# ApproximateCaesar/AlphaQuoridorGNN

Hardware: AMD Instinct MI355X
Metric: self-play games/sec, 9x9 Quoridor (PV-MCTS, GNN evaluator), whole job (higher is better)
Workload: dtype f32 (f16x3-split MFMA products, f32 accumulate); 1 GPU; BASELINE configs[2]/[3]: one self-play generation per step (lock-step PV-MCTS, random-weight GNN) + all-gather of (s,pi,z); games_per_gpu=2048, game_sets_per_gpu=4, sims_per_move=200, board=9x9, walls=10, plies_for_draw=116, parallelism=games sharded over 1 rank(s), 1 all-gather per generation

## Files before the change

### alphaquoridorgnn_amd/csrc/gcn_heads_split.hpp

```cpp
#pragma once
#include "gcn_packed.hpp"
#include <cmath>

namespace aqg {

__device__ __forceinline__ float row16_sum(float x) {
    x += __builtin_bit_cast(float, __builtin_amdgcn_update_dpp(0, __builtin_bit_cast(int, x), 0x128, 0xf, 0xf, false));
    x += __builtin_bit_cast(float, __builtin_amdgcn_update_dpp(0, __builtin_bit_cast(int, x), 0x124, 0xf, 0xf, false));
    x += __builtin_bit_cast(float, __builtin_amdgcn_update_dpp(0, __builtin_bit_cast(int, x), 0x122, 0xf, 0xf, false));
    x += __builtin_bit_cast(float, __builtin_amdgcn_update_dpp(0, __builtin_bit_cast(int, x), 0x121, 0xf, 0xf, false));
    return x;
}

__device__ __forceinline__ __amdgpu_buffer_rsrc_t packed_rsrc(const float* pk) {
    return __builtin_amdgcn_make_buffer_rsrc(const_cast<float*>(pk), 0, (int)(PackedLayout::TOTAL * sizeof(float)), 0x00020000);
}
__device__ __forceinline__ u32x4 load_frag16(__amdgpu_buffer_rsrc_t rs, int lane16, int byte_off) {
    return __builtin_amdgcn_raw_buffer_load_b128(rs, lane16, byte_off, 0);
}

__device__ __forceinline__ void report_saturation(bool lane_saw_it, int32_t* __restrict__ saturated) {
    if (saturated && __builtin_amdgcn_ballot_w64(lane_saw_it) != 0) {
        int l;
        asm volatile("v_mbcnt_lo_u32_b32 %0, -1, 0\n\tv_mbcnt_hi_u32_b32 %0, -1, %0" : "=v"(l));
        if (l == 0) atomicOr(saturated, 1);
    }
}

__device__ __forceinline__ void split8(const f32x4 x0, const f32x4 x1, u32x4& hi, u32x4& lo) {
    hi = (u32x4){cvt_pk_f16(x0[0], x0[1]), cvt_pk_f16(x0[2], x0[3]), cvt_pk_f16(x1[0], x1[1]), cvt_pk_f16(x1[2], x1[3])};
    const f32x4 r0 = x0 - f16_pairs_to_f32(hi[0], hi[1]), r1 = x1 - f16_pairs_to_f32(hi[2], hi[3]);
    lo = (u32x4){cvt_pk_f16(r0[0], r0[1]), cvt_pk_f16(r0[2], r0[3]), cvt_pk_f16(r1[0], r1[1]), cvt_pk_f16(r1[2], r1[3])};
}
__device__ __forceinline__ float row16_max(float x) {
    x = fmaxf(x, __builtin_bit_cast(float, __builtin_amdgcn_update_dpp(0, __builtin_bit_cast(int, x), 0x128, 0xf, 0xf, false)));
    x = fmaxf(x, __builtin_bit_cast(float, __builtin_amdgcn_update_dpp(0, __builtin_bit_cast(int, x), 0x124, 0xf, 0xf, false)));
    x = fmaxf(x, __builtin_bit_cast(float, __builtin_amdgcn_update_dpp(0, __builtin_bit_cast(int, x), 0x122, 0xf, 0xf, false)));
    x = fmaxf(x, __builtin_bit_cast(float, __builtin_amdgcn_update_dpp(0, __builtin_bit_cast(int, x), 0x121, 0xf, 0xf, false)));
    return x;
}

constexpr int HEADS_WAVES = 8;
struct alignas(16) HeadsSmem {
    unsigned int hfrag[2][2][64][4];
    float vlane[4][64];
    float wmax[HEADS_WAVES][16], wsum[HEADS_WAVES][16];
};

struct HeadsNoMid { __device__ __forceinline__ void operator()() const {} };
template <bool STEP = false, class Mid = HeadsNoMid>
__device__ __forceinline__ void heads_body(HeadsSmem& sm, __amdgpu_buffer_rsrc_t prs, int b0, int B, int A, __amdgpu_buffer_rsrc_t rs,
                                           const float* __restrict__ pk, float* __restrict__ logits, float* __restrict__ policy,
                                           float* __restrict__ value_pre, float* __restrict__ value, const uint8_t* __restrict__ active,
                                           int32_t* __restrict__ saturated, int wave, int lane, float (*lds_policy)[256] = nullptr,
                                           float* lds_value = nullptr, Mid mid = Mid()) {
    const int c = lane & 15, q = lane >> 4;
    constexpr int H1 = (int)(PackedLayout::WHH1 * sizeof(float)), P2 = (int)(PackedLayout::WHP2 * sizeof(float));
    const int ntiles = (A + 15) >> 4;
    const bool want_policy = STEP || logits || policy;
    u32x4 af[2][4];
#pragma unroll
    for (int pl = 0; pl < 2; ++pl)
#pragma unroll
        for (int kb = 0; kb < 4; ++kb) af[pl][kb] = load_frag16(rs, lane * 16, H1 + ((pl * 8 + wave) * 4 + kb) * (64 * 16));
    const bool okc = b0 + c < B;
    f32x4 x0[4], x1[4];
    {
        const int row = (okc ? b0 + c : B - 1) * (HID * 4);
#pragma unroll
        for (int kb = 0; kb < 4; ++kb) {
            x0[kb] = __builtin_bit_cast(f32x4, __builtin_amdgcn_raw_buffer_load_b128(prs, row + (32 * kb + 8 * q) * 4, 0, 0));
            x1[kb] = __builtin_bit_cast(f32x4, __builtin_amdgcn_raw_buffer_load_b128(prs, row + (32 * kb + 8 * q + 4) * 4, 0, 0));
        }
    }
    const f32x4 bias = *reinterpret_cast<const f32x4*>(pk + PackedLayout::HB1 + 16 * wave + 4 * q);
    const f32x4 vw = *reinterpret_cast<const f32x4*>(pk + PackedLayout::VW2 + 16 * (wave & 3) + 4 * q);
    float pb[2];
#pragma unroll
    for (int j = 0; j < 2; ++j) { const int a = 16 * (wave + 8 * j) + c; pb[j] = pk[PackedLayout::PB2 + (a < A ? a : 0)]; }
    const float vb2 = pk[PackedLayout::VB2];
    const uint8_t* __restrict__ ap = active ? active : reinterpret_cast<const uint8_t*>(pk);
    unsigned int af4[4];
#pragma unroll
    for (int i = 0; i < 4; ++i) af4[i] = ap[active ? min(b0 + 4 * q + i, B - 1) : 0];
    const unsigned int afc = ap[active ? min(b0 + c, B - 1) : 0];
    u32x4 ph[4], pl_[4];
    bool counted;
    {
        float xmax = 0.f;
#pragma unroll
        for (int kb = 0; kb < 4; ++kb) {
            if (!okc) { x0[kb] = (f32x4){0.f, 0.f, 0.f, 0.f}; x1[kb] = x0[kb]; }
#pragma unroll
            for (int e = 0; e < 4; ++e) xmax = fmaxf(fmaxf(fabsf(x0[kb][e]), fabsf(x1[kb][e])), xmax);
            split8(x0[kb], x1[kb], ph[kb], pl_[kb]);
        }
        counted = okc && (!active || (STEP ? afc == 1 : afc != 0));
        if (wave == 0) report_saturation(counted && !(xmax <= 65504.0f), saturated);
    }
    int live4 = 0;
#pragma unroll
    for (int i = 0; i < 4; ++i) live4 |= (b0 + 4 * q + i < B && (!active || (STEP ? af4[i] == 1 : af4[i] != 0))) ? (1 << i) : 0;
    u32x4 bq[2][2][2];
    auto request_bq = [&](int j, int kb) {
        const int at = wave + 8 * j;
#pragma unroll
        for (int pl = 0; pl < 2; ++pl)
            bq[j][pl][kb] = (want_policy && at < ntiles) ? load_frag16(rs, lane * 16, P2 + ((pl * 14 + at) * 2 + kb) * (64 * 16)) : (u32x4){0u, 0u, 0u, 0u};
    };
    if (!STEP) {
#pragma unroll
        for (int j = 0; j < 2; ++j)
#pragma unroll
            for (int kb = 0; kb < 2; ++kb) request_bq(j, kb);
    }
    {
        f32x4 acc = (f32x4){0.f, 0.f, 0.f, 0.f};
#pragma unroll
        for (int kb = 0; kb < 4; ++kb) {
            acc = mfma_f16(af[1][kb], ph[kb], acc);
            acc = mfma_f16(af[0][kb], pl_[kb], acc);
            acc = mfma_f16(af[0][kb], ph[kb], acc);
            if (STEP) {
                __builtin_amdgcn_sched_barrier(0);
                request_bq(kb >> 1, kb & 1);
                __builtin_amdgcn_sched_barrier(0);
            }
        }
        if (STEP) {
            __builtin_amdgcn_sched_barrier(0);
            mid();
            __builtin_amdgcn_sched_barrier(0);
        }
        f32x4 h = acc + bias;
#pragma unroll
        for (int e = 0; e < 4; ++e) h[e] = fmaxf(h[e], 0.f);
        if (wave < 4) {
            report_saturation(counted && !(fmaxf(fmaxf(h[0], h[1]), fmaxf(h[2], h[3])) <= 65504.0f), saturated);
            const unsigned int h01 = cvt_pk_f16(h[0], h[1]), h23 = cvt_pk_f16(h[2], h[3]);
            const f32x4 r = h - f16_pairs_to_f32(h01, h23);
            const int kb2 = wave >> 1, t = wave & 1;
            *reinterpret_cast<u32x2*>(&sm.hfrag[kb2][0][lane][2 * t]) = (u32x2){h01, h23};
            *reinterpret_cast<u32x2*>(&sm.hfrag[kb2][1][lane][2 * t]) = (u32x2){cvt_pk_f16(r[0], r[1]), cvt_pk_f16(r[2], r[3])};
        } else {
            sm.vlane[wave - 4][lane] = h[0] * vw[0] + h[1] * vw[1] + h[2] * vw[2] + h[3] * vw[3];
        }
    }
    __syncthreads();
    if (wave == 4) {
        float v = (sm.vlane[0][lane] + sm.vlane[1][lane]) + (sm.vlane[2][lane] + sm.vlane[3][lane]);
        v += __shfl_xor(v, 16);
        v += __shfl_xor(v, 32);
        if (counted && lane < 16) {
            v += vb2;
            if (STEP) lds_value[lane] = tanhf(v);
            else {
                if (value_pre) value_pre[b0 + lane] = v;
                if (value) value[b0 + lane] = tanhf(v);
            }
        }
    }
    if (!want_policy) return;
    u32x4 hh[2], hl[2];
#pragma unroll
    for (int kb = 0; kb < 2; ++kb) {
        hh[kb] = *reinterpret_cast<const u32x4*>(&sm.hfrag[kb][0][lane][0]);
        hl[kb] = *reinterpret_cast<const u32x4*>(&sm.hfrag[kb][1][lane][0]);
    }
    f32x4 lg[2];
    f32x4 m = (f32x4){-INFINITY, -INFINITY, -INFINITY, -INFINITY};
#pragma unroll
    for (int j = 0; j < 2; ++j) {
        const int at = wave + 8 * j, a = 16 * at + c;
        f32x4 acc = (f32x4){0.f, 0.f, 0.f, 0.f};
#pragma unroll
        for (int kb = 0; kb < 2; ++kb) {
            acc = mfma_f16(hl[kb], bq[j][0][kb], acc);
            acc = mfma_f16(hh[kb], bq[j][1][kb], acc);
            acc = mfma_f16(hh[kb], bq[j][0][kb], acc);
        }
        const bool ok = a < A;
#pragma unroll
        for (int i = 0; i < 4; ++i) {
            lg[j][i] = ok ? acc[i] + pb[j] : -INFINITY;
            m[i] = fmaxf(m[i], lg[j][i]);
        }
    }
    f32x4 ssum = (f32x4){0.f, 0.f, 0.f, 0.f};
    f32x4 ex[2];
#pragma unroll
    for (int i = 0; i < 4; ++i) m[i] = row16_max(m[i]);
#pragma unroll
    for (int j = 0; j < 2; ++j)
#pragma unroll
        for (int i = 0; i < 4; ++i) {
            ex[j][i] = __expf(lg[j][i] - m[i]);
            ssum[i] += ex[j][i];
        }
#pragma unroll
    for (int i = 0; i < 4; ++i) ssum[i] = row16_sum(ssum[i]);
    if (c == 0) {
        *reinterpret_cast<f32x4*>(&sm.wmax[wave][4 * q]) = m;
        *reinterpret_cast<f32x4*>(&sm.wsum[wave][4 * q]) = ssum;
    }
    __syncthreads();
    f32x4 scale;
    {
        int qo = 4 * q;
        f32x4 M = (f32x4){-INFINITY, -INFINITY, -INFINITY, -INFINITY};
#pragma unroll
        for (int w = 0; w < HEADS_WAVES; ++w) {
            const f32x4 mw = *reinterpret_cast<const f32x4*>(&sm.wmax[w][qo]);
#pragma unroll
            for (int i = 0; i < 4; ++i) M[i] = fmaxf(M[i], mw[i]);
        }
        f32x4 S = (f32x4){0.f, 0.f, 0.f, 0.f};
#pragma unroll
        for (int w = 0; w < HEADS_WAVES; ++w) {
            if (STEP && (w & 3) == 0) {
                const float d0 = w ? S[0] : M[0], d1 = w ? S[1] : M[1], d2 = w ? S[2] : M[2], d3 = w ? S[3] : M[3];
                asm volatile("" : "+v"(qo) : "v"(d0), "v"(d1), "v"(d2), "v"(d3));
            }
            const f32x4 mw = *reinterpret_cast<const f32x4*>(&sm.wmax[w][qo]);
            const f32x4 sw = *reinterpret_cast<const f32x4*>(&sm.wsum[w][qo]);
#pragma unroll
            for (int i = 0; i < 4; ++i) S[i] += sw[i] * __expf(mw[i] - M[i]);
        }
#pragma unroll
        for (int i = 0; i < 4; ++i) scale[i] = __expf(m[i] - M[i]) / S[i];
    }
#pragma unroll
    for (int i = 0; i < 4; ++i) {
        const int brd = b0 + 4 * q + i;
        if (!((live4 >> i) & 1)) continue;
        if (STEP) {
            float* p = &lds_policy[4 * q + i][16 * wave + c];
#pragma unroll
            for (int j = 0; j < 2; ++j) if (16 * (wave + 8 * j) + c < A) p[128 * j] = ex[j][i] * scale[i];
            continue;
        }
        const size_t row = (size_t)brd * A + 16 * wave + c;
        if (policy) {
            float* __restrict__ p = policy + row;
#pragma unroll
            for (int j = 0; j < 2; ++j) if (16 * (wave + 8 * j) + c < A) p[128 * j] = ex[j][i] * scale[i];
        }
        if (logits) {
            float* __restrict__ l = logits + row;
#pragma unroll
            for (int j = 0; j < 2; ++j) if (16 * (wave + 8 * j) + c < A) l[128 * j] = lg[j][i];
        }
    }
}

}
```

### alphaquoridorgnn_amd/csrc/mcts.hip

```cpp
#define AQG_TRACE_TU mcts
#include "aqg_common.hpp"
#include <vector>
#include <cstring>
#include "legal_wave.hpp"
#include "../../include/aqgnn.h"
#include "launchers.hpp"
#include "counter_rng.hpp"
#include "gcn_heads_split.hpp"
#include <cfloat>

#pragma clang fp contract(off)

namespace aqg {

int g_use_graph = 1;

__device__ __forceinline__ int wave_sum_i(int v) {
#pragma unroll
    for (int off = 32; off > 0; off >>= 1) v += __shfl_xor(v, off);
    return v;
}
__device__ __forceinline__ float wave_sum_f(float v) {
#pragma unroll
    for (int off = 32; off > 0; off >>= 1) v += __shfl_xor(v, off);
// ... 158 lines not shown
    const uint8_t* ord = e.legal_order + (size_t)g * MAX_LEGAL;
    const int prow = s.ppos / N;
    int rl[3]; int tot = 0;
#pragma unroll
    for (int r = 0; r < 3; ++r) {
        const int i = lane + 64 * r;
        rl[r] = 0;
        if (i < cnt) {
            const int a = ord[i];
            uint32_t x = ((h ^ ((uint32_t)(a + 1) * 0x9E3779B1u)) * 0x85EBCA6Bu) >> 22;
            int rr = (int)x + 1;
            if (a < V && (a / N) < prow) rr *= 1 + e.fake_bias;
            rl[r] = rr; tot += rr;
        }
    }
    tot = wave_sum_i(tot);
    float* pol = e.policy + (size_t)g * A;
#pragma unroll
    for (int r = 0; r < 3; ++r) {
        const int i = lane + 64 * r;
        if (i < cnt) pol[i] = (float)rl[r] / (float)tot;
    }
    if (lane == 0) e.value[g] = (float)((int)((h * 0xC2B2AE35u) >> 16) - 32768) / 32768.0f;
}

#ifdef AQG_STAMP
#define STEP_STAMP_DECL unsigned long long sp_prev = __builtin_readcyclecounter(), sp_loc[5] = {0, 0, 0, 0, 0};
#define STEP_STAMP(i) { const unsigned long long sp_now = __builtin_readcyclecounter(); if (lane == 0) reinterpret_cast<unsigned long long*>(e.pooled + (size_t)g * 128)[i] += sp_now - sp_prev; sp_loc[i] = sp_now - sp_prev; sp_prev = sp_now; }
#define LEVEL_STAMP(i) { const unsigned long long lv_now = __builtin_readcyclecounter(); if (lane == 0) reinterpret_cast<unsigned long long*>(e.pooled + (size_t)g * 128)[i] += lv_now - lv_prev; lv_prev = lv_now; }
#else
#define STEP_STAMP_DECL
#define STEP_STAMP(i)
#endif
constexpr int EVAL_CACHE_ROW = 704;
static_assert(MAX_LEGAL * 5 <= EVAL_CACHE_ROW && MAX_LEGAL % 4 == 0, "evaluation cache row");
__device__ __forceinline__ uint32_t eval_cache_misc(const QState& s) {
    return (uint32_t)s.ppos | ((uint32_t)s.pwl << 8) | ((uint32_t)s.epos << 16) | ((uint32_t)s.ewl << 24);
}

int g_step_prio = 1;
int g_step_waves = 8;
int g_step_fast_depth = 61;
int g_step_heads = 1;

__device__ __forceinline__ QState state_of_words(uint64_t q0, uint64_t q1, uint64_t m) {
    QState s;
    s.hw = q0; s.vw = q1;
    s.ppos = (uint8_t)(m & 0xff); s.pwl = (uint8_t)((m >> 8) & 0xff);
    s.epos = (uint8_t)((m >> 16) & 0xff); s.ewl = (uint8_t)((m >> 24) & 0xff);
    s.plies = (uint16_t)((m >> 32) & 0xffff); s.pad = 0;
    return s;
}

struct StepRound1 {
    int active, flag, depth_old, cnt_new, first_new, cslot, pnode;
    float value;
    uint64_t root_q0, root_q1, root_q2, leaf_q0, leaf_q1, leaf_q2;
    uint32_t oa0, oa1, oa2;
    float polr0, polr1, polr2, polr3;
    NodeRec rootrec;
    u32x4 hot0, hot1, hot2, cold0, cold1, cold2;
};
template <int N, bool CACHE, bool HEADS>
__device__ __forceinline__ void step_round1(const aqg_engine& e, int g, int lane, int do_expand, StepRound1& r1) {
    constexpr int A = Geo<N>::A;
    const NodeRec* __restrict__ nodes = game_nodes(e, g);
    const int* path = e.path + (size_t)g * (e.sims + 2);
    const uint8_t* ord = e.legal_order + (size_t)g * MAX_LEGAL;
    const float* pol = e.policy + (size_t)g * A;
    r1.active = e.game_active[g];
    const uint64_t* rq = reinterpret_cast<const uint64_t*>(e.root_state) + (size_t)g * 3;
    r1.root_q0 = rq[0]; r1.root_q1 = rq[1]; r1.root_q2 = rq[2];
    int flag = 0, depth_old = 0, cnt_new = 0, first_new = 0, cslot = -1, pnode = 0;
    float value = 0.f;
    uint32_t oa[3] = {0u, 0u, 0u};
    float polr[4] = {0.f, 0.f, 0.f, 0.f};
    r1.leaf_q0 = r1.leaf_q1 = r1.leaf_q2 = 0;
    if (HEADS) {
        flag = e.leaf_flag[g]; depth_old = e.path_len[g]; cnt_new = e.legal_count[g]; first_new = e.node_count[g]; value = e.value[g];
        if (CACHE) {
            cslot = e.eval_cache_slot[g];
            const uint64_t* lq = reinterpret_cast<const uint64_t*>(e.leaf_state) + (size_t)g * 3;
            r1.leaf_q0 = lq[0]; r1.leaf_q1 = lq[1]; r1.leaf_q2 = lq[2];
        }
        static_assert(!HEADS || MAX_LEGAL <= A, "the legal-ordered row fits the dense one");
        static_assert(128 < MAX_LEGAL && MAX_LEGAL <= 192, "lane rounds 0 and 1 lie inside the legal list, round 2 is masked by the consumer");
#pragma unroll
        for (int r = 0; r < 3; ++r) { const int i = min(lane + 64 * r, MAX_LEGAL - 1); oa[r] = (uint32_t)ord[i]; polr[r] = pol[i]; }
        pnode = path[min(lane, e.sims + 1)];
    } else if (do_expand) {
        flag = e.leaf_flag[g]; depth_old = e.path_len[g]; cnt_new = e.legal_count[g]; first_new = e.node_count[g]; value = e.value[g];
        if (CACHE) {
            cslot = e.eval_cache_slot[g];
            const uint64_t* lq = reinterpret_cast<const uint64_t*>(e.leaf_state) + (size_t)g * 3;
            r1.leaf_q0 = lq[0]; r1.leaf_q1 = lq[1]; r1.leaf_q2 = lq[2];
        }
#pragma unroll
        for (int r = 0; r < 3; ++r) { const int i = lane + 64 * r; oa[r] = (i < MAX_LEGAL) ? (uint32_t)ord[i] : 0u; }
        pnode = (lane < e.sims + 2) ? path[lane] : 0;
        if (e.prior_mode == 0) {
#pragma unroll
            for (int r = 0; r < 4; ++r) { const int a = lane + 64 * r; polr[r] = (a < A) ? pol[a] : 0.f; }
        } else {
#pragma unroll
            for (int r = 0; r < 3; ++r) { const int i = lane + 64 * r; polr[r] = (i < MAX_LEGAL && i < A) ? pol[i] : 0.f; }
        }
    }
    r1.flag = flag; r1.depth_old = depth_old; r1.cnt_new = cnt_new; r1.first_new = first_new; r1.cslot = cslot; r1.pnode = pnode; r1.value = value;
    r1.oa0 = oa[0]; r1.oa1 = oa[1]; r1.oa2 = oa[2];
    r1.polr0 = polr[0]; r1.polr1 = polr[1]; r1.polr2 = polr[2]; r1.polr3 = polr[3];
    r1.rootrec = nodes[0];
    const u32x4* __restrict__ nhalf = reinterpret_cast<const u32x4*>(nodes);
    u32x4 hot[3], cold[3];
#pragma unroll
    for (int r = 0; r < 3; ++r) {
        const int i = min(1 + lane + 64 * r, e.node_cap - 1);
        cold[r] = nhalf[2 * i]; hot[r] = nhalf[2 * i + 1];
    }
    r1.hot0 = hot[0]; r1.hot1 = hot[1]; r1.hot2 = hot[2]; r1.cold0 = cold[0]; r1.cold1 = cold[1]; r1.cold2 = cold[2];
}

template <int N, bool CACHE, bool HEADS>
__device__ __forceinline__ void game_step_fast(const aqg_engine& e, int g, int lane, int do_expand, int do_select, int fast_depth,
                                               float* __restrict__ polbuf , int list_sim,
                                               const StepRound1& r1, float head_value) {
    constexpr int A = Geo<N>::A;
    NodeRec* __restrict__ nodes = game_nodes(e, g);
    int* path = e.path + (size_t)g * (e.sims + 2);
    STEP_STAMP_DECL
    const int active = r1.active;
    const QState s_loaded = state_of_words(r1.root_q0, r1.root_q1, r1.root_q2);
    int flag = r1.flag, depth_old = r1.depth_old, cnt_new = r1.cnt_new, first_new = r1.first_new;
    float value = r1.value;
    const uint8_t oa[3] = {(uint8_t)r1.oa0, (uint8_t)r1.oa1, (uint8_t)((HEADS && lane + 128 >= MAX_LEGAL) ? 0u : r1.oa2)};
    const int pnode = (HEADS && lane >= e.sims + 2) ? 0 : r1.pnode;
    const float polr[4] = {r1.polr0, r1.polr1, r1.polr2, r1.polr3};
    constexpr bool cache_on = CACHE;
    int cslot = r1.cslot;
    const QState leaf_prev = (cache_on && do_expand) ? state_of_words(r1.leaf_q0, r1.leaf_q1, r1.leaf_q2) : s_loaded;
    const NodeRec rootrec = r1.rootrec;
    const u32x4* __restrict__ nhalf = reinterpret_cast<const u32x4*>(nodes);
    u32x4 hot[3] = {r1.hot0, r1.hot1, r1.hot2}, cold[3] = {r1.cold0, r1.cold1, r1.cold2};
    if (!do_expand) flag = 0;
    flag = __builtin_amdgcn_readfirstlane(flag); depth_old = __builtin_amdgcn_readfirstlane(depth_old);
    cnt_new = __builtin_amdgcn_readfirstlane(cnt_new); first_new = __builtin_amdgcn_readfirstlane(first_new);
    const bool hit_old = flag == 2;
    if (hit_old) flag = 1;
    if (HEADS && !hit_old) value = head_value;
    if (flag != 1 && !do_select) return;
#ifdef AQG_STAMP
    asm volatile("s_waitcnt vmcnt(0)" ::: "memory");
#endif
    STEP_STAMP(0)

    const bool expanded = flag == 1 && cnt_new > 0 && first_new + cnt_new <= e.node_cap;
    const int leaf_old = flag == 1 ? (depth_old < 64 ? __builtin_amdgcn_readlane(pnode, depth_old & 63) : path[depth_old]) : -1;
    float pl[3] = {0.f, 0.f, 0.f};
    if (flag == 1) {
        if (e.prior_mode == 0 && !hit_old) {
            if (!HEADS) {
#pragma unroll
                for (int r = 0; r < 4; ++r) polbuf[lane + 64 * r] = polr[r];
                __builtin_amdgcn_fence(__ATOMIC_RELEASE, "wavefront");
                __builtin_amdgcn_wave_barrier();
                __builtin_amdgcn_fence(__ATOMIC_ACQUIRE, "wavefront");
            }
            float sum = 0.f;
#pragma unroll
            for (int r = 0; r < 3; ++r) {
                const int i = lane + 64 * r;
                pl[r] = (i < cnt_new) ? polbuf[oa[r]] : 0.f;
                sum += pl[r];
            }
            sum = wave_sum_f(sum);
            const float den = (sum != 0.f) ? sum : 1.f;
#pragma unroll
            for (int r = 0; r < 3; ++r) pl[r] = pl[r] / den;
        } else {
#pragma unroll
            for (int r = 0; r < 3; ++r) { const int i = lane + 64 * r; pl[r] = (i < cnt_new) ? polr[r] : 0.f; }
        }
        if (cache_on && !hit_old) {
            cslot = __builtin_amdgcn_readfirstlane(cslot);
            if (cslot >= 0) {
                const size_t ent = ((size_t)g << e.eval_cache_log2) + (size_t)cslot;
                unsigned char* row = reinterpret_cast<unsigned char*>(e.eval_cache_rows) + ent * EVAL_CACHE_ROW;
                float* rp = reinterpret_cast<float*>(row);
                uint8_t* ro = row + MAX_LEGAL * sizeof(float);
#pragma unroll
                for (int r = 0; r < 3; ++r) {
                    const int i = lane + 64 * r;
                    if (i < MAX_LEGAL) { rp[i] = pl[r]; ro[i] = (i < cnt_new) ? oa[r] : (uint8_t)0xFF; }
                }
                if (lane == 0) {
                    const QState k = uniform_state(leaf_prev);
                    u32x4* kr = reinterpret_cast<u32x4*>(e.eval_cache_keys) + 2 * ent;
                    kr[0] = (u32x4){(uint32_t)k.hw, (uint32_t)(k.hw >> 32), (uint32_t)k.vw, (uint32_t)(k.vw >> 32)};
                    kr[1] = (u32x4){eval_cache_misc(k), 2u, (uint32_t)cnt_new, __builtin_bit_cast(uint32_t, value)};
                }
            }
        }
        if (expanded) {
#pragma unroll
            for (int r = 0; r < 3; ++r) {
                const int i = lane + 64 * r;
                if (i < cnt_new) {
                    NodeRec c;
                    c.w = 0.0; c.p = pl[r]; c.n = 0; c.kids = 0; c.action = oa[r]; c.q = 0.f; c.cp = e.c_puct * pl[r];
                    nodes[first_new + i] = c;
                }
            }
            if (lane == 0) {
                nodes[leaf_old].kids = (uint32_t)first_new | ((uint32_t)cnt_new << 24);
                e.node_count[g] = first_new + cnt_new;
            }
        }
        if (lane == 0) e.stat_leaf_evals[g] += 1;
    }
    const uint32_t kids_new = expanded ? ((uint32_t)first_new | ((uint32_t)cnt_new << 24)) : 0u;
    const double v_old = (double)value;
    double bw = 0.0; int bn = 0;
    float bq = 0.f;
    const bool fast_old = flag == 1 && depth_old <= fast_depth && depth_old < 63;
    if (flag == 1 && fast_old) {
        if (lane <= depth_old) {
            const NodeRec& r = nodes[pnode];
            bw = r.w + (((depth_old - lane) & 1) ? -v_old : v_old);
            bn = r.n + 1;
            bq = q_of(bw, bn);
        }
    }
    bool pending = fast_old;
    auto flush_old = [&]() {
        if (pending && lane <= depth_old) { NodeRec& r = nodes[pnode]; r.w = bw; r.n = bn; r.q = bq; }
        pending = false;
    };
    if (flag == 1 && !fast_old) {
        if (lane <= depth_old && lane < 64) {
            NodeRec& r = nodes[pnode];
            r.w += ((depth_old - lane) & 1) ? -v_old : v_old;
            r.n += 1;
            r.q = q_of(r.w, r.n);
// ... 72 lines not shown
        if (m0) bi = __builtin_ctzll(m0);
        else if (cnt > 64) {
            const uint64_t v1 = cnt >= 128 ? ~0ull : ((1ull << (cnt - 64)) - 1ull);
            const uint64_t m1 = __ballot(sc[1] == best) & v1;
            if (m1) bi = 64 + __builtin_ctzll(m1);
            else if (cnt > 128) {
                const uint64_t m2 = __ballot(sc[2] == best) & ((1ull << (cnt - 128)) - 1ull);
                if (m2) bi = 128 + __builtin_ctzll(m2);
            }
        }
        besti = __builtin_amdgcn_readfirstlane(bi);
        const int slot = besti >> 6, src = besti & 63;
        uint32_t wlo, whi;
        auto pick = [&](const u32x4 c, uint32_t k, int n) {
            const uint32_t c0 = c[0], c1 = c[1], c3 = c[3];
            kids_n = (uint32_t)__builtin_amdgcn_readlane((int)k, src);
            action = __builtin_amdgcn_readlane((int)c3, src);
            cn = __builtin_amdgcn_readlane(n, src);
            wlo = (uint32_t)__builtin_amdgcn_readlane((int)c0, src);
            whi = (uint32_t)__builtin_amdgcn_readlane((int)c1, src);
        };
        if (slot == 0) pick(cold[0], keff[0], neff[0]); else if (slot == 1) pick(cold[1], keff[1], neff[1]); else pick(cold[2], keff[2], neff[2]);
        cw = __builtin_bit_cast(double, ((uint64_t)whi << 32) | wlo);
        node = first + besti;
        onpath = patch && besti == pidx;
#pragma unroll
        for (int r = 0; r < 3; ++r) asm volatile("" :: "v"(hot[r]), "v"(cold[r]));
    };
    auto stop_here = [&]() -> int {
        const bool lose = is_lose<N>(s), draw = is_draw(s, e.plies_for_draw);
        if (lose || draw) { tvalue = lose ? -1.0 : 0.0; terminal = 1; return 1; }
        if ((kids >> 24) == 0) return 2;
        if (regs && onpath && depth == depth_old) return 3;
        return 0;
    };
    bool at_old_leaf = false;
#ifdef AQG_STAMP_LEVELS
    unsigned long long lv_prev = __builtin_readcyclecounter();
#endif
    int stop = stop_here();
    if (stop == 0) {
        if (!regs) {
#pragma unroll
            for (int r = 0; r < 3; ++r) {
                const int i = (int)(kids & 0xFFFFFF) + max(min(lane + 64 * r, (int)(kids >> 24) - 1), 0);
                cold[r] = nhalf[2 * i]; hot[r] = nhalf[2 * i + 1];
            }
        }
        select_level(hot, cold);
#ifdef AQG_STAMP_LEVELS
        lv_prev = __builtin_readcyclecounter();
#endif
        for (;;) {
            if (regs && depth + 1 >= fast_depth) {
                flush_old();
                __builtin_amdgcn_fence(__ATOMIC_RELEASE, "workgroup");
                __builtin_amdgcn_wave_barrier();
                __builtin_amdgcn_fence(__ATOMIC_ACQUIRE, "workgroup");
                regs = false;
                onpath = false;
            }
            u32x4 h[3], c[3];
#ifdef AQG_STAMP_LEVELS
            LEVEL_STAMP(11)
#endif
            {
// ... 60 lines not shown
                r.n += 1;
                r.q = q_of(r.w, r.n);
            }
        }
        if (lane == 0) {
            e.stat_terminal_sims[g] += 1;
            for (int d = 64; d <= depth; ++d) {
                NodeRec& r = nodes[path[d]];
                r.w += ((depth - d) & 1) ? -tvalue : tvalue;
                r.n += 1;
                r.q = q_of(r.w, r.n);
            }
        }
    } else {
        flush_old();
        bool hit = false;
        int newslot = -1;
        LegalPrep prep;
        if (!cache_on) prep = wave_legal_prepare<N>(s, lane);
        if (cache_on) {
            const uint32_t misc = eval_cache_misc(s);
            uint64_t h = s.hw * 0x9E3779B97F4A7C15ull ^ s.vw * 0xC2B2AE3D27D4EB4Full ^ (uint64_t)misc * 0x165667B19E3779F9ull;
            h ^= h >> 29; h *= 0xBF58476D1CE4E5B9ull; h ^= h >> 32;
            const uint32_t cmask = (1u << e.eval_cache_log2) - 1u, home = (uint32_t)h & cmask;
            const size_t base = (size_t)g << e.eval_cache_log2;
            const u32x4* keys = reinterpret_cast<const u32x4*>(e.eval_cache_keys) + 2 * base;
            const uint32_t idx = (home + (uint32_t)lane) & cmask;
            const u32x4 k0 = keys[2 * idx], k1 = keys[2 * idx + 1];
            prep = wave_legal_prepare<N>(s, lane);
            const uint32_t a0 = k0[0], a1 = k0[1], a2 = k0[2], a3 = k0[3], b0 = k1[0], b1 = k1[1], b2 = k1[2], b3 = k1[3];
            const bool match = a0 == (uint32_t)s.hw && a1 == (uint32_t)(s.hw >> 32) && a2 == (uint32_t)s.vw && a3 == (uint32_t)(s.vw >> 32) &&
                               b0 == misc && b1 == 2u;
            const uint64_t mb = __ballot(match);
            if (mb) {
                hit = true;
                const int src = __builtin_ctzll(mb);
                const uint32_t hs = (home + (uint32_t)src) & cmask;
                const int cnt = __builtin_amdgcn_readlane((int)b2, src);
                const uint32_t vbits = (uint32_t)__builtin_amdgcn_readlane((int)b3, src);
                const unsigned char* row = reinterpret_cast<const unsigned char*>(e.eval_cache_rows) + (base + hs) * EVAL_CACHE_ROW;
                const float* rp = reinterpret_cast<const float*>(row);
                float* pdst = e.policy + (size_t)g * A;
#pragma unroll
                for (int r = 0; r < 3; ++r) { const int i = lane + 64 * r; if (i < cnt) pdst[i] = rp[i]; }
                if (lane < MAX_LEGAL / 4)
                    reinterpret_cast<uint32_t*>(e.legal_order + (size_t)g * MAX_LEGAL)[lane] = reinterpret_cast<const uint32_t*>(row + MAX_LEGAL * sizeof(float))[lane];
                STEP_STAMP(3)
                if (lane == 0) {
                    store_state(e.leaf_state, g, s);
                    e.legal_count[g] = cnt;
                    e.path_len[g] = depth;
                    e.value[g] = __builtin_bit_cast(float, vbits);
                    e.leaf_flag[g] = 2;
                    e.stat_cache_hits[g] += 1;
                }
            } else {
                const uint64_t eb = __ballot(b1 == 0u);
                newslot = (int)((home + (uint32_t)(eb ? __builtin_ctzll(eb) : (int)((h >> 40) & 63u))) & cmask);
            }
        }
        if (!hit) {
            const int total = wave_legal_finish<N>(s, prep, lane, nullptr, e.legal_order + (size_t)g * MAX_LEGAL);
            STEP_STAMP(3)
            if (lane == 0) {
                store_state(e.leaf_state, g, s);
                e.legal_count[g] = total;
                e.path_len[g] = depth;
                e.leaf_flag[g] = 1;
                if (cache_on) {
                    e.eval_mask[g] = 1; e.eval_cache_slot[g] = newslot;
                    if (list_sim >= 0) e.eval_list[atomicAdd(e.eval_count + list_sim, 1)] = g;
                }
            }
        }
    }
#ifdef AQG_STAMP
    asm volatile("s_waitcnt vmcnt(0)" ::: "memory");
    STEP_STAMP(4)
    if (lane == 0) {
        unsigned long long* o = reinterpret_cast<unsigned long long*>(e.pooled + (size_t)g * 128);
        o[7] += 1;
        const unsigned long long tot = sp_loc[0] + sp_loc[1] + sp_loc[2] + sp_loc[3] + sp_loc[4];
        if (tot > o[16]) { o[16] = tot; for (int i = 0; i < 5; ++i) o[17 + i] = sp_loc[i]; o[22] = (unsigned long long)depth; o[23] = (unsigned long long)terminal; }
        const unsigned long long bk = tot >> 11;
        o[24 + (bk < 39 ? bk : 39)] += 1;
    }
#endif
}

template <int N, bool CACHE, bool HEADS>
__global__ __launch_bounds__(512, HEADS ? 4 : 1) void engine_step_fast_kernel(aqg_engine e, int do_expand, int do_select, int fast_depth, int list_sim) {
    __shared__ float polbuf[8][256];
    AQG_TRACE_BEGIN
    const int lane = threadIdx.x & 63;
    const int g = blockIdx.x * (blockDim.x >> 6) + (threadIdx.x >> 6);
    { const int pr = (fast_depth >> 8) & 3; if (pr == 1) __builtin_amdgcn_s_setprio(1); else if (pr == 2) __builtin_amdgcn_s_setprio(2); else if (pr == 3) __builtin_amdgcn_s_setprio(3); }
    fast_depth &= 0xFF;
    StepRound1 r1;
    if constexpr (HEADS) {
        __shared__ HeadsSmem hsm;
        __shared__ float hval[16];
        const int wave = __builtin_amdgcn_readfirstlane(threadIdx.x >> 6);
        const int b0 = blockIdx.x * 8, bend = min(e.num_games, b0 + 8);
        const __amdgpu_buffer_rsrc_t prs = __builtin_amdgcn_make_buffer_rsrc(e.pooled, 0, e.num_games * (HID * 4), 0x00020000);
        heads_body<true>(hsm, prs, b0, bend, Geo<N>::A, packed_rsrc(e.packed_weights), e.packed_weights, nullptr, nullptr, nullptr, nullptr,
                         e.leaf_flag, e.counters + 5, wave, lane, polbuf, hval,
                         [&]() { step_round1<N, CACHE, true>(e, min(g, e.num_games - 1), lane, 1, r1); });
        __syncthreads();
        if (g < e.num_games) game_step_fast<N, CACHE, true>(e, g, lane, do_expand, do_select, fast_depth, polbuf[wave], list_sim, r1, hval[wave]);
    } else if (g < e.num_games) {
        step_round1<N, CACHE, false>(e, g, lane, do_expand, r1);
        game_step_fast<N, CACHE, false>(e, g, lane, do_expand, do_select, fast_depth, polbuf[threadIdx.x >> 6], list_sim, r1, 0.f);
    }
    AQG_TRACE_END(1, (unsigned long long)(uintptr_t)e.pooled)
}
AQG_TRACE_SETTER(set_trace_mcts)

template <int N>
static void launch_step(const aqg_engine& e_in, int do_expand, int do_select, hipStream_t st, int list_sim = -1, bool heads = false) {
    aqg_engine e = e_in;
    if (e.prior_mode == 3 || e.prior_mode == 4) e.prior_mode = 0;
    if (g_profile_trunk == 2) profile_mark(st, e.num_games);
    const int wpb = (g_step_waves == 1 || g_step_waves == 2 || g_step_waves == 8) ? g_step_waves : 4;
    const int fd = g_step_fast_depth | ((g_step_prio & 3) << 8);
    const dim3 sg((e.num_games + wpb - 1) / wpb), sb(64 * wpb);
    const bool cache = e.eval_cache_keys && e.prior_mode == 0;
    if (!cache) list_sim = -1;
    bool fused = false;
    if constexpr (N == 9) fused = heads && do_expand && wpb == 8 && e.prior_mode == 0;
    auto launch = [&](auto kernel) { hipLaunchKernelGGL(kernel, sg, sb, 0, st, e, do_expand, do_select, fd, list_sim); };
    if constexpr (N == 9) {
        if (fused) { if (cache) launch(engine_step_fast_kernel<N, true, true>); else launch(engine_step_fast_kernel<N, false, true>); }
    }
    if (!fused) { if (cache) launch(engine_step_fast_kernel<N, true, false>); else launch(engine_step_fast_kernel<N, false, false>); }
    if (g_profile_trunk == 2) profile_mark(st, -1);
}

constexpr int ROOT_NOISE_ATTEMPTS = 64;
__device__ __forceinline__ double wave_sum_d(double v) {
#pragma unroll
    for (int off = 32; off > 0; off >>= 1) v += __shfl_xor(v, off);
    return v;
}
__device__ __forceinline__ double root_noise_gamma(uint64_t key, double alpha) {
    const bool boost = alpha < 1.0;
    const double a = boost ? alpha + 1.0 : alpha;
    const double d = a - 1.0 / 3.0, c = 1.0 / sqrt(9.0 * d);
    double val = d;
    for (int t = 0; t < ROOT_NOISE_ATTEMPTS; ++t) {
// ... 450 lines not shown
```

Before: 1234 games/s.

## Defer fused policy-head softmax to a single tail wave after tree selection

In the fused heads+step kernel, the policy head (second matmul, softmax, prior write) is pulled off the critical path. Waves now compute only the hidden layer and value, run selection and expansion with placeholder priors, and the first wave to finish computes all 8 games' policies. That wave renormalizes them and writes the priors into the new child nodes and the eval-cache rows. Round-1 loads are split into two parts so they can be interleaved around the hidden matmul, and self-hits on the game's own cache entry are treated specially. The risk is that selection in the same step reads children whose priors are not yet written (guarded by returning at the old leaf), and a single wave serializes eight policy computations.

```diff
diff --git a/alphaquoridorgnn_amd/csrc/gcn_heads_split.hpp b/alphaquoridorgnn_amd/csrc/gcn_heads_split.hpp
--- a/alphaquoridorgnn_amd/csrc/gcn_heads_split.hpp
+++ b/alphaquoridorgnn_amd/csrc/gcn_heads_split.hpp
@@ -47,17 +47,16 @@
     float wmax[HEADS_WAVES][16], wsum[HEADS_WAVES][16];
 };
 
-struct HeadsNoMid { __device__ __forceinline__ void operator()() const {} };
+struct HeadsNoMid { __device__ __forceinline__ void operator()(int) const {} };
 template <bool STEP = false, class Mid = HeadsNoMid>
 __device__ __forceinline__ void heads_body(HeadsSmem& sm, __amdgpu_buffer_rsrc_t prs, int b0, int B, int A, __amdgpu_buffer_rsrc_t rs,
                                            const float* __restrict__ pk, float* __restrict__ logits, float* __restrict__ policy,
                                            float* __restrict__ value_pre, float* __restrict__ value, const uint8_t* __restrict__ active,
-                                           int32_t* __restrict__ saturated, int wave, int lane, float (*lds_policy)[256] = nullptr,
-                                           float* lds_value = nullptr, Mid mid = Mid()) {
+                                           int32_t* __restrict__ saturated, int wave, int lane, Mid mid = Mid()) {
     const int c = lane & 15, q = lane >> 4;
     constexpr int H1 = (int)(PackedLayout::WHH1 * sizeof(float)), P2 = (int)(PackedLayout::WHP2 * sizeof(float));
     const int ntiles = (A + 15) >> 4;
-    const bool want_policy = STEP || logits || policy;
+    const bool want_policy = logits || policy;
     u32x4 af[2][4];
 #pragma unroll
     for (int pl = 0; pl < 2; ++pl)
@@ -75,15 +74,24 @@
     }
     const f32x4 bias = *reinterpret_cast<const f32x4*>(pk + PackedLayout::HB1 + 16 * wave + 4 * q);
     const f32x4 vw = *reinterpret_cast<const f32x4*>(pk + PackedLayout::VW2 + 16 * (wave & 3) + 4 * q);
-    float pb[2];
-#pragma unroll
-    for (int j = 0; j < 2; ++j) { const int a = 16 * (wave + 8 * j) + c; pb[j] = pk[PackedLayout::PB2 + (a < A ? a : 0)]; }
-    const float vb2 = pk[PackedLayout::VB2];
+    float pb[2] = {0.f, 0.f};
+    if (!STEP) {
+#pragma unroll
+        for (int j = 0; j < 2; ++j) { const int a = 16 * (wave + 8 * j) + c; pb[j] = pk[PackedLayout::PB2 + (a < A ? a : 0)]; }
+    }
+    const float vb2 = STEP ? 0.f : pk[PackedLayout::VB2];
     const uint8_t* __restrict__ ap = active ? active : reinterpret_cast<const uint8_t*>(pk);
-    unsigned int af4[4];
-#pragma unroll
-    for (int i = 0; i < 4; ++i) af4[i] = ap[active ? min(b0 + 4 * q + i, B - 1) : 0];
+    unsigned int af4[4] = {0u, 0u, 0u, 0u};
+    if (!STEP) {
+#pragma unroll
+        for (int i = 0; i < 4; ++i) af4[i] = ap[active ? min(b0 + 4 * q + i, B - 1) : 0];
+    }
     const unsigned int afc = ap[active ? min(b0 + c, B - 1) : 0];
+    if (STEP) {
+        __builtin_amdgcn_sched_barrier(0);
+        mid(0);
+        __builtin_amdgcn_sched_barrier(0);
+    }
     u32x4 ph[4], pl_[4];
     bool counted;
     {
@@ -100,7 +108,7 @@
     }
     int live4 = 0;
 #pragma unroll
-    for (int i = 0; i < 4; ++i) live4 |= (b0 + 4 * q + i < B && (!active || (STEP ? af4[i] == 1 : af4[i] != 0))) ? (1 << i) : 0;
+    for (int i = 0; i < 4; ++i) live4 |= (b0 + 4 * q + i < B && (!active || af4[i] != 0)) ? (1 << i) : 0;
     u32x4 bq[2][2][2];
     auto request_bq = [&](int j, int kb) {
         const int at = wave + 8 * j;
@@ -121,15 +129,10 @@
             acc = mfma_f16(af[1][kb], ph[kb], acc);
             acc = mfma_f16(af[0][kb], pl_[kb], acc);
             acc = mfma_f16(af[0][kb], ph[kb], acc);
-            if (STEP) {
-                __builtin_amdgcn_sched_barrier(0);
-                request_bq(kb >> 1, kb & 1);
-                __builtin_amdgcn_sched_barrier(0);
-            }
         }
         if (STEP) {
             __builtin_amdgcn_sched_barrier(0);
-            mid();
+            mid(1);
             __builtin_amdgcn_sched_barrier(0);
         }
         f32x4 h = acc + bias;
@@ -146,6 +149,7 @@
             sm.vlane[wave - 4][lane] = h[0] * vw[0] + h[1] * vw[1] + h[2] * vw[2] + h[3] * vw[3];
         }
     }
+    if (STEP) return;
     __syncthreads();
     if (wave == 4) {
         float v = (sm.vlane[0][lane] + sm.vlane[1][lane]) + (sm.vlane[2][lane] + sm.vlane[3][lane]);
@@ -153,11 +157,8 @@
         v += __shfl_xor(v, 32);
         if (counted && lane < 16) {
             v += vb2;
-            if (STEP) lds_value[lane] = tanhf(v);
-            else {
-                if (value_pre) value_pre[b0 + lane] = v;
-                if (value) value[b0 + lane] = tanhf(v);
-            }
+            if (value_pre) value_pre[b0 + lane] = v;
+            if (value) value[b0 + lane] = tanhf(v);
         }
     }
     if (!want_policy) return;
@@ -206,7 +207,7 @@
     __syncthreads();
     f32x4 scale;
     {
-        int qo = 4 * q;
+        const int qo = 4 * q;
         f32x4 M = (f32x4){-INFINITY, -INFINITY, -INFINITY, -INFINITY};
 #pragma unroll
         for (int w = 0; w < HEADS_WAVES; ++w) {
@@ -217,10 +218,6 @@
         f32x4 S = (f32x4){0.f, 0.f, 0.f, 0.f};
 #pragma unroll
         for (int w = 0; w < HEADS_WAVES; ++w) {
-            if (STEP && (w & 3) == 0) {
-                const float d0 = w ? S[0] : M[0], d1 = w ? S[1] : M[1], d2 = w ? S[2] : M[2], d3 = w ? S[3] : M[3];
-                asm volatile("" : "+v"(qo) : "v"(d0), "v"(d1), "v"(d2), "v"(d3));
-            }
             const f32x4 mw = *reinterpret_cast<const f32x4*>(&sm.wmax[w][qo]);
             const f32x4 sw = *reinterpret_cast<const f32x4*>(&sm.wsum[w][qo]);
 #pragma unroll
@@ -233,12 +230,6 @@
     for (int i = 0; i < 4; ++i) {
         const int brd = b0 + 4 * q + i;
         if (!((live4 >> i) & 1)) continue;
-        if (STEP) {
-            float* p = &lds_policy[4 * q + i][16 * wave + c];
-#pragma unroll
-            for (int j = 0; j < 2; ++j) if (16 * (wave + 8 * j) + c < A) p[128 * j] = ex[j][i] * scale[i];
-            continue;
-        }
         const size_t row = (size_t)brd * A + 16 * wave + c;
         if (policy) {
             float* __restrict__ p = policy + row;
@@ -253,4 +244,120 @@
     }
 }
 
-}
+__device__ __forceinline__ float heads_step_value(const HeadsSmem& sm, const float* __restrict__ pk, int lane, int i) {
+    const float vb2 = pk[PackedLayout::VB2];
+    float v = (sm.vlane[0][lane] + sm.vlane[1][lane]) + (sm.vlane[2][lane] + sm.vlane[3][lane]);
+    v += __shfl_xor(v, 16);
+    v += __shfl_xor(v, 32);
+    v += vb2;
+    return __builtin_bit_cast(float, __builtin_amdgcn_readlane(__builtin_bit_cast(int, tanhf(v)), i));
+}
+
+__device__ __forceinline__ void heads_policy_tail(HeadsSmem& sm, int A, __amdgpu_buffer_rsrc_t rs, const float* __restrict__ pk, int lane,
+                                                  float (*lds_policy)[256]) {
+    const int c = lane & 15, q = lane >> 4;
+    constexpr int P2 = (int)(PackedLayout::WHP2 * sizeof(float));
+    const int ntiles = (A + 15) >> 4;
+    u32x4 hh[2], hl[2];
+#pragma unroll
+    for (int kb = 0; kb < 2; ++kb) {
+        hh[kb] = *reinterpret_cast<const u32x4*>(&sm.hfrag[kb][0][lane][0]);
+        hl[kb] = *reinterpret_cast<const u32x4*>(&sm.hfrag[kb][1][lane][0]);
+    }
+#pragma unroll
+    for (int w = 0; w < HEADS_WAVES; ++w) {
+        u32x4 bq[2][2][2];
+        float pb[2];
+#pragma unroll
+        for (int j = 0; j < 2; ++j) {
+            const int at = w + 8 * j, a = 16 * at + c;
+#pragma unroll
+            for (int kb = 0; kb < 2; ++kb)
+#pragma unroll
+                for (int pl = 0; pl < 2; ++pl)
+                    bq[j][pl][kb] = at < ntiles ? load_frag16(rs, lane * 16, P2 + ((pl * 14 + at) * 2 + kb) * (64 * 16)) : (u32x4){0u, 0u, 0u, 0u};
+            pb[j] = pk[PackedLayout::PB2 + (a < A ? a : 0)];
+        }
+        f32x4 lg[2];
+        f32x4 m = (f32x4){-INFINITY, -INFINITY, -INFINITY, -INFINITY};
+#pragma unroll
+        for (int j = 0; j < 2; ++j) {
+            const int at = w + 8 * j, a = 16 * at + c;
+            f32x4 acc = (f32x4){0.f, 0.f, 0.f, 0.f};
+#pragma unroll
+            for (int kb = 0; kb < 2; ++kb) {
+                acc = mfma_f16(hl[kb], bq[j][0][kb], acc);
+                acc = mfma_f16(hh[kb], bq[j][1][kb], acc);
+                acc = mfma_f16(hh[kb], bq[j][0][kb], acc);
+            }
+            const bool ok = a < A;
+#pragma unroll
+            for (int i = 0; i < 4; ++i) {
+                lg[j][i] = ok ? acc[i] + pb[j] : -INFINITY;
+                m[i] = fmaxf(m[i], lg[j][i]);
+            }
+        }
+        f32x4 ssum = (f32x4){0.f, 0.f, 0.f, 0.f};
+        f32x4 ex[2];
+#pragma unroll
+        for (int i = 0; i < 4; ++i) m[i] = row16_max(m[i]);
+#pragma unroll
+        for (int j = 0; j < 2; ++j)
+#pragma unroll
+            for (int i = 0; i < 4; ++i) {
+                ex[j][i] = __expf(lg[j][i] - m[i]);
+                ssum[i] += ex[j][i];
+            }
+#pragma unroll
+        for (int i = 0; i < 4; ++i) ssum[i] = row16_sum(ssum[i]);
+        if (c == 0) {
+            *reinterpret_cast<f32x4*>(&sm.wmax[w][4 * q]) = m;
+            *reinterpret_cast<f32x4*>(&sm.wsum[w][4 * q]) = ssum;
+        }
+        if (q < 2) {
+#pragma unroll
+            for (int i = 0; i < 4; ++i)
+#pragma unroll
+                for (int j = 0; j < 2; ++j) if (16 * (w + 8 * j) + c < A) lds_policy[4 * q + i][16 * (w + 8 * j) + c] = ex[j][i];
+        }
+    }
+    __builtin_amdgcn_fence(__ATOMIC_RELEASE, "wavefront");
+    __builtin_amdgcn_wave_barrier();
+    __builtin_amdgcn_fence(__ATOMIC_ACQUIRE, "wavefront");
+    const int qo = 4 * q;
+    f32x4 M = (f32x4){-INFINITY, -INFINITY, -INFINITY, -INFINITY};
+#pragma unroll
+    for (int w = 0; w < HEADS_WAVES; ++w) {
+        const f32x4 mw = *reinterpret_cast<const f32x4*>(&sm.wmax[w][qo]);
+#pragma unroll
+        for (int i = 0; i < 4; ++i) M[i] = fmaxf(M[i], mw[i]);
+    }
+    f32x4 S = (f32x4){0.f, 0.f, 0.f, 0.f};
+#pragma unroll
+    for (int w = 0; w < HEADS_WAVES; ++w) {
+        const f32x4 mw = *reinterpret_cast<const f32x4*>(&sm.wmax[w][qo]);
+        const f32x4 sw = *reinterpret_cast<const f32x4*>(&sm.wsum[w][qo]);
+#pragma unroll
+        for (int i = 0; i < 4; ++i) S[i] += sw[i] * __expf(mw[i] - M[i]);
+    }
+    if (q < 2) {
+#pragma unroll
+        for (int w = 0; w < HEADS_WAVES; ++w) {
+            const f32x4 m = *reinterpret_cast<const f32x4*>(&sm.wmax[w][qo]);
+            f32x4 scale;
+#pragma unroll
+            for (int i = 0; i < 4; ++i) scale[i] = __expf(m[i] - M[i]) / S[i];
+#pragma unroll
+            for (int i = 0; i < 4; ++i) {
+                float* p = &lds_policy[4 * q + i][16 * w + c];
+#pragma unroll
+                for (int j = 0; j < 2; ++j) if (16 * (w + 8 * j) + c < A) p[128 * j] = p[128 * j] * scale[i];
+            }
+        }
+    }
+    __builtin_amdgcn_fence(__ATOMIC_RELEASE, "wavefront");
+    __builtin_amdgcn_wave_barrier();
+    __builtin_amdgcn_fence(__ATOMIC_ACQUIRE, "wavefront");
+}
+
+}
diff --git a/alphaquoridorgnn_amd/csrc/mcts.hip b/alphaquoridorgnn_amd/csrc/mcts.hip
--- a/alphaquoridorgnn_amd/csrc/mcts.hip
+++ b/alphaquoridorgnn_amd/csrc/mcts.hip
@@ -214,6 +214,9 @@
 #define STEP_STAMP_DECL
 #define STEP_STAMP(i)
 #endif
+#ifdef AQG_STAMP_HEADS
+static __device__ unsigned long long g_stamp_heads[16];
+#endif
 constexpr int EVAL_CACHE_ROW = 704;
 static_assert(MAX_LEGAL * 5 <= EVAL_CACHE_ROW && MAX_LEGAL % 4 == 0, "evaluation cache row");
 __device__ __forceinline__ uint32_t eval_cache_misc(const QState& s) {
@@ -244,9 +247,10 @@
     u32x4 hot0, hot1, hot2, cold0, cold1, cold2;
 };
 template <int N, bool CACHE, bool HEADS>
-__device__ __forceinline__ void step_round1(const aqg_engine& e, int g, int lane, int do_expand, StepRound1& r1) {
+__device__ __forceinline__ void step_round1(const aqg_engine& e, int g, int lane, int do_expand, StepRound1& r1, int parts = 3) {
     constexpr int A = Geo<N>::A;
     const NodeRec* __restrict__ nodes = game_nodes(e, g);
+    if (parts & 1) {
     const int* path = e.path + (size_t)g * (e.sims + 2);
     const uint8_t* ord = e.legal_order + (size_t)g * MAX_LEGAL;
     const float* pol = e.policy + (size_t)g * A;
@@ -292,6 +296,8 @@
     r1.oa0 = oa[0]; r1.oa1 = oa[1]; r1.oa2 = oa[2];
     r1.polr0 = polr[0]; r1.polr1 = polr[1]; r1.polr2 = polr[2]; r1.polr3 = polr[3];
     r1.rootrec = nodes[0];
+    }
+    if (!(parts & 2)) return;
     const u32x4* __restrict__ nhalf = reinterpret_cast<const u32x4*>(nodes);
     u32x4 hot[3], cold[3];
 #pragma unroll
@@ -300,6 +306,20 @@
         cold[r] = nhalf[2 * i]; hot[r] = nhalf[2 * i + 1];
     }
     r1.hot0 = hot[0]; r1.hot1 = hot[1]; r1.hot2 = hot[2]; r1.cold0 = cold[0]; r1.cold1 = cold[1]; r1.cold2 = cold[2];
+}
+
+__device__ __forceinline__ void gather_renorm(const float* __restrict__ row, const uint8_t (&oa)[3], int cnt, int lane, float (&pl)[3]) {
+    float sum = 0.f;
+#pragma unroll
+    for (int r = 0; r < 3; ++r) {
+        const int i = lane + 64 * r;
+        pl[r] = (i < cnt) ? row[oa[r]] : 0.f;
+        sum += pl[r];
+    }
+    sum = wave_sum_f(sum);
+    const float den = (sum != 0.f) ? sum : 1.f;
+#pragma unroll
+    for (int r = 0; r < 3; ++r) pl[r] = pl[r] / den;
 }
 
 template <int N, bool CACHE, bool HEADS>
@@ -328,6 +348,7 @@
     cnt_new = __builtin_amdgcn_readfirstlane(cnt_new); first_new = __builtin_amdgcn_readfirstlane(first_new);
     const bool hit_old = flag == 2;
     if (hit_old) flag = 1;
+    const bool tail_priors = HEADS && !hit_old;
     if (HEADS && !hit_old) value = head_value;
     if (flag != 1 && !do_select) return;
 #ifdef AQG_STAMP
@@ -338,6 +359,7 @@
     const bool expanded = flag == 1 && cnt_new > 0 && first_new + cnt_new <= e.node_cap;
     const int leaf_old = flag == 1 ? (depth_old < 64 ? __builtin_amdgcn_readlane(pnode, depth_old & 63) : path[depth_old]) : -1;
     float pl[3] = {0.f, 0.f, 0.f};
+    int own_ent = -1;
     if (flag == 1) {
         if (e.prior_mode == 0 && !hit_old) {
             if (!HEADS) {
@@ -346,24 +368,15 @@
                 __builtin_amdgcn_fence(__ATOMIC_RELEASE, "wavefront");
                 __builtin_amdgcn_wave_barrier();
                 __builtin_amdgcn_fence(__ATOMIC_ACQUIRE, "wavefront");
-            }
-            float sum = 0.f;
-#pragma unroll
-            for (int r = 0; r < 3; ++r) {
-                const int i = lane + 64 * r;
-                pl[r] = (i < cnt_new) ? polbuf[oa[r]] : 0.f;
-                sum += pl[r];
-            }
-            sum = wave_sum_f(sum);
-            const float den = (sum != 0.f) ? sum : 1.f;
-#pragma unroll
-            for (int r = 0; r < 3; ++r) pl[r] = pl[r] / den;
+                gather_renorm(polbuf, oa, cnt_new, lane, pl);
+            }
         } else {
 #pragma unroll
             for (int r = 0; r < 3; ++r) { const int i = lane + 64 * r; pl[r] = (i < cnt_new) ? polr[r] : 0.f; }
         }
         if (cache_on && !hit_old) {
             cslot = __builtin_amdgcn_readfirstlane(cslot);
+            if (tail_priors) own_ent = cslot;
             if (cslot >= 0) {
                 const size_t ent = ((size_t)g << e.eval_cache_log2) + (size_t)cslot;
                 unsigned char* row = reinterpret_cast<unsigned char*>(e.eval_cache_rows) + ent * EVAL_CACHE_ROW;
@@ -372,7 +385,7 @@
 #pragma unroll
                 for (int r = 0; r < 3; ++r) {
                     const int i = lane + 64 * r;
-                    if (i < MAX_LEGAL) { rp[i] = pl[r]; ro[i] = (i < cnt_new) ? oa[r] : (uint8_t)0xFF; }
+                    if (i < MAX_LEGAL) { if (!tail_priors) rp[i] = pl[r]; ro[i] = (i < cnt_new) ? oa[r] : (uint8_t)0xFF; }
                 }
                 if (lane == 0) {
                     const QState k = uniform_state(leaf_prev);
@@ -387,9 +400,14 @@
             for (int r = 0; r < 3; ++r) {
                 const int i = lane + 64 * r;
                 if (i < cnt_new) {
-                    NodeRec c;
-                    c.w = 0.0; c.p = pl[r]; c.n = 0; c.kids = 0; c.action = oa[r]; c.q = 0.f; c.cp = e.c_puct * pl[r];
-                    nodes[first_new + i] = c;
+                    if (tail_priors) {
+                        NodeRec& c = nodes[first_new + i];
+                        c.w = 0.0; c.action = oa[r]; c.n = 0; c.kids = 0; c.q = 0.f;
+                    } else {
+                        NodeRec c;
+                        c.w = 0.0; c.p = pl[r]; c.n = 0; c.kids = 0; c.action = oa[r]; c.q = 0.f; c.cp = e.c_puct * pl[r];
+                        nodes[first_new + i] = c;
+                    }
                 }
             }
             if (lane == 0) {
@@ -528,6 +546,7 @@
         if (lose || draw) { tvalue = lose ? -1.0 : 0.0; terminal = 1; return 1; }
         if ((kids >> 24) == 0) return 2;
         if (regs && onpath && depth == depth_old) return 3;
+        if (HEADS && node == leaf_old) return 3;
         return 0;
     };
     bool at_old_leaf = false;
@@ -654,7 +673,10 @@
             const bool match = a0 == (uint32_t)s.hw && a1 == (uint32_t)(s.hw >> 32) && a2 == (uint32_t)s.vw && a3 == (uint32_t)(s.vw >> 32) &&
                                b0 == misc && b1 == 2u;
             const uint64_t mb = __ballot(match);
-            if (mb) {
+            const bool own = HEADS && mb && own_ent >= 0 && ((home + (uint32_t)__builtin_ctzll(mb)) & cmask) == (uint32_t)own_ent;
+            if (own) {
+                if (lane == 0) e.stat_cache_hits[g] += 1;
+            } else if (mb) {
                 hit = true;
                 const int src = __builtin_ctzll(mb);
                 const uint32_t hs = (home + (uint32_t)src) & cmask;
@@ -710,6 +732,52 @@
 #endif
 }
 
+struct StepTailSmem {
+    uint8_t ord[8][MAX_LEGAL];
+    int meta[8][4];
+    unsigned int ticket;
+};
+template <int N, bool CACHE>
+__device__ __forceinline__ void step_policy_tail(const aqg_engine& e, int b0, int lane, HeadsSmem& hsm, float (*polbuf)[256], const StepTailSmem& tsm) {
+    heads_policy_tail(hsm, Geo<N>::A, packed_rsrc(e.packed_weights), e.packed_weights, lane, polbuf);
+#ifdef AQG_STAMP_HEADS
+    const unsigned long long hs_g0 = __builtin_amdgcn_s_memrealtime();
+    unsigned long long hs_games = 0;
+#endif
+    for (int w = 0; w < 8; ++w) {
+        const int flag = __builtin_amdgcn_readfirstlane(tsm.meta[w][0]), cnt_new = __builtin_amdgcn_readfirstlane(tsm.meta[w][1]);
+        const int first_new = __builtin_amdgcn_readfirstlane(tsm.meta[w][2]), cslot = __builtin_amdgcn_readfirstlane(tsm.meta[w][3]);
+        if (flag != 1) continue;
+        const int g = b0 + w;
+        uint8_t oa[3];
+#pragma unroll
+        for (int r = 0; r < 3; ++r) { const int i = lane + 64 * r; oa[r] = i < MAX_LEGAL ? tsm.ord[w][i] : (uint8_t)0; }
+        float pl[3];
+        gather_renorm(polbuf[w], oa, cnt_new, lane, pl);
+        if (cnt_new > 0 && first_new + cnt_new <= e.node_cap) {
+            NodeRec* __restrict__ nodes = game_nodes(e, g);
+#pragma unroll
+            for (int r = 0; r < 3; ++r) {
+                const int i = lane + 64 * r;
+                if (i < cnt_new) { NodeRec& c = nodes[first_new + i]; c.p = pl[r]; c.cp = e.c_puct * pl[r]; }
+            }
+        }
+        if (CACHE && cslot >= 0) {
+            const size_t ent = ((size_t)g << e.eval_cache_log2) + (size_t)cslot;
+            float* rp = reinterpret_cast<float*>(reinterpret_cast<unsigned char*>(e.eval_cache_rows) + ent * EVAL_CACHE_ROW);
+#pragma unroll
+            for (int r = 0; r < 3; ++r) { const int i = lane + 64 * r; if (i < MAX_LEGAL) rp[i] = pl[r]; }
+        }
+#ifdef AQG_STAMP_HEADS
+        hs_games += 1;
+#endif
+    }
+#ifdef AQG_STAMP_HEADS
+    asm volatile("s_waitcnt vmcnt(0)" ::: "memory");
+    if (lane == 0) { atomicAdd(&g_stamp_heads[3], hs_games); atomicAdd(&g_stamp_heads[4], __builtin_amdgcn_s_memrealtime() - hs_g0); }
+#endif
+}
+
 template <int N, bool CACHE, bool HEADS>
 __global__ __launch_bounds__(512, HEADS ? 4 : 1) void engine_step_fast_kernel(aqg_engine e, int do_expand, int do_select, int fast_depth, int list_sim) {
     __shared__ float polbuf[8][256];
@@ -721,15 +789,68 @@
     StepRound1 r1;
     if constexpr (HEADS) {
         __shared__ HeadsSmem hsm;
-        __shared__ float hval[16];
+        __shared__ StepTailSmem tsm;
         const int wave = __builtin_amdgcn_readfirstlane(threadIdx.x >> 6);
         const int b0 = blockIdx.x * 8, bend = min(e.num_games, b0 + 8);
         const __amdgpu_buffer_rsrc_t prs = __builtin_amdgcn_make_buffer_rsrc(e.pooled, 0, e.num_games * (HID * 4), 0x00020000);
+#ifdef AQG_STAMP_HEADS
+        __shared__ unsigned long long hs_t[5][8];
+        const unsigned long long hs_t0 = __builtin_amdgcn_s_memrealtime();
+#endif
+        if (threadIdx.x == 0) tsm.ticket = 0u;
         heads_body<true>(hsm, prs, b0, bend, Geo<N>::A, packed_rsrc(e.packed_weights), e.packed_weights, nullptr, nullptr, nullptr, nullptr,
-                         e.leaf_flag, e.counters + 5, wave, lane, polbuf, hval,
-                         [&]() { step_round1<N, CACHE, true>(e, min(g, e.num_games - 1), lane, 1, r1); });
+                         e.leaf_flag, e.counters + 5, wave, lane,
+                         [&](int part) { step_round1<N, CACHE, true>(e, min(g, e.num_games - 1), lane, 1, r1, 1 << part); });
+        {
+#pragma unroll
+            for (int r = 0; r < 3; ++r) {
+                const int i = lane + 64 * r;
+                if (i < MAX_LEGAL) tsm.ord[wave][i] = (uint8_t)(r == 0 ? r1.oa0 : (r == 1 ? r1.oa1 : r1.oa2));
+            }
+            if (lane == 0) {
+                tsm.meta[wave][0] = g < e.num_games ? r1.flag : 0; tsm.meta[wave][1] = r1.cnt_new;
+                tsm.meta[wave][2] = r1.first_new; tsm.meta[wave][3] = r1.cslot;
+            }
+        }
         __syncthreads();
-        if (g < e.num_games) game_step_fast<N, CACHE, true>(e, g, lane, do_expand, do_select, fast_depth, polbuf[wave], list_sim, r1, hval[wave]);
+#ifdef AQG_STAMP_HEADS
+        const unsigned long long hs_t1 = __builtin_amdgcn_s_memrealtime();
+#endif
+        if (g < e.num_games) {
+            const float hv = heads_step_value(hsm, e.packed_weights, lane, wave);
+            game_step_fast<N, CACHE, true>(e, g, lane, do_expand, do_select, fast_depth, polbuf[wave], list_sim, r1, hv);
+        }
+#ifdef AQG_STAMP_HEADS
+        asm volatile("s_waitcnt vmcnt(0)" ::: "memory");
+        if (lane == 0) { hs_t[0][wave] = hs_t0; hs_t[1][wave] = hs_t1; hs_t[2][wave] = __builtin_amdgcn_s_memrealtime(); hs_t[3][wave] = 0; hs_t[4][wave] = 0; }
+#endif
+        unsigned int ticket = 0u;
+        if (lane == 0) ticket = atomicAdd(&tsm.ticket, 1u);
+        ticket = (unsigned int)__builtin_amdgcn_readfirstlane((int)ticket);
+        if (ticket == 0u) {
+#ifdef AQG_STAMP_HEADS
+            const unsigned long long hs_a = __builtin_amdgcn_s_memrealtime();
+#endif
+            step_policy_tail<N, CACHE>(e, b0, lane, hsm, polbuf, tsm);
+#ifdef AQG_STAMP_HEADS
+            asm volatile("s_waitcnt vmcnt(0)" ::: "memory");
+            if (lane == 0) { hs_t[3][wave] = hs_a; hs_t[4][wave] = __builtin_amdgcn_s_memrealtime(); }
+#endif
+        }
+#ifdef AQG_STAMP_HEADS
+        __syncthreads();
+        if (threadIdx.x == 0) {
+            unsigned long long beg = hs_t[0][0], en[8], bar = 0, ta = 0, tb = 0;
+            for (int w = 0; w < 8; ++w) beg = hs_t[0][w] < beg ? hs_t[0][w] : beg;
+            for (int w = 0; w < 8; ++w) { en[w] = hs_t[2][w] - beg; bar += hs_t[1][w] - beg; if (hs_t[4][w]) { ta = hs_t[3][w]; tb = hs_t[4][w]; } }
+            for (int i = 1; i < 8; ++i) for (int j = i; j > 0 && en[j] < en[j - 1]; --j) { const unsigned long long t = en[j]; en[j] = en[j - 1]; en[j - 1] = t; }
+            atomicAdd(&g_stamp_heads[0], 1ull); atomicAdd(&g_stamp_heads[1], 8ull);
+            atomicAdd(&g_stamp_heads[5], en[0]); atomicAdd(&g_stamp_heads[6], (en[3] + en[4]) / 2); atomicAdd(&g_stamp_heads[7], en[7]);
+            atomicAdd(&g_stamp_heads[8], bar / 8);
+            atomicAdd(&g_stamp_heads[9], 1ull); atomicAdd(&g_stamp_heads[10], tb - ta); atomicAdd(&g_stamp_heads[11], tb - beg);
+            if (tb - beg > en[7]) atomicAdd(&g_stamp_heads[12], 1ull);
+        }
+#endif
     } else if (g < e.num_games) {
         step_round1<N, CACHE, false>(e, g, lane, do_expand, r1);
         game_step_fast<N, CACHE, false>(e, g, lane, do_expand, do_select, fast_depth, polbuf[threadIdx.x >> 6], list_sim, r1, 0.f);
@@ -737,6 +858,16 @@
     AQG_TRACE_END(1, (unsigned long long)(uintptr_t)e.pooled)
 }
 AQG_TRACE_SETTER(set_trace_mcts)
+#ifdef AQG_STAMP_HEADS
+}
+extern "C" int aqg_stamp_heads_read(unsigned long long* out16, int reset) {
+    if (hipDeviceSynchronize() != hipSuccess) return -1;
+    if (hipMemcpyFromSymbol(out16, HIP_SYMBOL(aqg::g_stamp_heads), 16 * sizeof(unsigned long long)) != hipSuccess) return -1;
+    if (reset) { unsigned long long z[16] = {}; if (hipMemcpyToSymbol(HIP_SYMBOL(aqg::g_stamp_heads), z, sizeof(z)) != hipSuccess) return -1; }
+    return 0;
+}
+namespace aqg {
+#endif
 
 template <int N>
 static void launch_step(const aqg_engine& e_in, int do_expand, int do_select, hipStream_t st, int list_sim = -1, bool heads = false) {
```

After: 1075 games/s. 0.871x the previous value.
